# marcinp7/music-style-transfer

Hardware: AMD Instinct MI355X
Metric: style-transfer opt iters/sec (higher is better)
Workload: dtype f32; 1 GPU; one 30 s clip per GPU (BASELINE.json configs[1]): piano-roll C=4,R=16,T=4 (+percussion), full widths (980325 params), fwd+loss+bwd every step, Adam+StepLR every iter_size steps; clips_per_gpu=1, iter_size=2, hip_graph=True, graphs=one joint graph, accumulation=2 concurrent streams, launches_per_pass=71, parallelism=single GPU

## Files before the change

music-style-transfer_amd/csrc/loss_optim.hip:

```cpp
#include "mst_common.h"

#define LOSS_MAXBLK 256
#define NP_SUMS 7
#define N_TAPE_IN 16
#define SAVED_J 0
#define EPS_DIV 1e-7f

int64_t mst_loss_scratch_floats(void) { return 2 * LOSS_MAXBLK * 8 + 64; }

template <int NFEAT>
__device__ __forceinline__ void note_terms(const float* p, const float* t, float* acc) {
    const float pv = p[1], tv = t[1];
    const float m = tv > 0.f ? 1.f : 0.f;
    acc[0] += fminf(pv, tv);
    acc[1] += fmaxf(pv - tv, 0.f);
    acc[2] += fmaxf(tv - pv, 0.f);
    const float dv = tv - pv;
    acc[3] += dv * dv * m;
    const float dd = (p[0] - fminf(t[0], 6.f)) / 6.f;
    acc[4] += dd * dd * m;
    if (NFEAT == 5) {
        float bce = 0.f;
#pragma unroll
        for (int a = 2; a < 5; ++a) {
            const float lp = fmaxf(logf(p[a]), -100.f), lq = fmaxf(logf(1.f - p[a]), -100.f);
            bce -= t[a] * lp + (1.f - t[a]) * lq;
        }
        acc[5] += bce * m;
    }
    acc[6] += m;
}
// ... 92 lines not shown

__device__ __forceinline__ ChannelLeaves channel_tree(const Dual* in, bool pitched, bool normalize) {
    const Dual TP = in[0], FP = in[1], FN = in[2], SEV = in[3], SED = in[4];
    const Dual NM = pitched ? in[6] : in[5];
    ChannelLeaves o;
    const Dual prec = d_safe_div(TP, d_add(TP, FP));
    const Dual rec = d_safe_div(TP, d_add(TP, FN));
    const Dual f = d_cmul(d_safe_div(d_mul(prec, rec), d_add(prec, rec)), 2.f);
    o.notes = d_one_minus(f);
    o.vel = d_div(SEV, NM);
    o.dur = d_div(SED, NM);
    const Dual nv = d_safe_sqrt(d_add(d_mul(o.notes, d_sqr(o.notes)), d_mul(d_one_minus(o.notes), d_sqr(o.vel))));
    if (pitched) {
        o.acc = d_div(in[5], d_cmul(NM, 3.f));
        if (normalize) o.acc = d_tanh(o.acc);
        o.total = d_qmean3(o.dur, o.acc, nv);
    } else {
        o.acc = dl(0.f, 0.f);
        o.total = d_qmean2(o.dur, nv);
    }
    return o;
}

__global__ __launch_bounds__(64) void loss_tail_kernel(const float* scratch, int nblk_p, int nblk_u, int has_u,
                                                       const float* il, const float* it, int ni,
                                                       const float* mlg, const float* mt,
                                                       const float* bp, const float* bt, int normalize,
                                                       float* losses, float* saved, LossBatch lb,
                                                       float* gl_onehot, float* losses_out) {
    __shared__ float sums[N_TAPE_IN];
    const int tid = threadIdx.x;
    {
        const int64_t k = blockIdx.y;
        scratch += k * lb.tmp; il += k * lb.ws; it += k * lb.ws; mlg += k * lb.ws; mt += k * lb.ws; bp += k * lb.ws;
        bt += k * lb.ws; losses += k * lb.ws; saved += k * lb.ws;
        if (gl_onehot) gl_onehot += k * lb.ws;
        if (losses_out) losses_out += k * MST_N_LOSSES;
    }
    {
        float sp[8] = {0.f, 0.f, 0.f, 0.f, 0.f, 0.f, 0.f, 0.f}, su[8] = {0.f, 0.f, 0.f, 0.f, 0.f, 0.f, 0.f, 0.f};
        typedef float row4 __attribute__((ext_vector_type(4), aligned(4)));
        const row4* rp = reinterpret_cast<const row4*>(scratch);
        const row4* ru = reinterpret_cast<const row4*>(scratch + LOSS_MAXBLK * 8);
        const int nbu = has_u ? nblk_u : 0;
        for (int q = tid; q < nblk_p; q += 64) {
            const row4 x = rp[2 * q], y = rp[2 * q + 1];
            sp[0] += x.x; sp[1] += x.y; sp[2] += x.z; sp[3] += x.w; sp[4] += y.x; sp[5] += y.y; sp[6] += y.z;
        }
        for (int q = tid; q < nbu; q += 64) {
            const row4 x = ru[2 * q], y = ru[2 * q + 1];
            su[0] += x.x; su[1] += x.y; su[2] += x.z; su[3] += x.w; su[4] += y.x; su[5] += y.y; su[6] += y.z;
        }
#pragma unroll
        for (int k = 0; k < 7; ++k) { sp[k] = wave_sum(sp[k]); su[k] = wave_sum(su[k]); }
        if (tid == 0) {
#pragma unroll
            for (int k = 0; k < 7; ++k) sums[k] = sp[k];
#pragma unroll
            for (int k = 0; k < 5; ++k) sums[7 + k] = su[k];
            sums[12] = su[6];
        }
    }
    float v = 0.f;
    for (int j = tid; j < ni; j += 64) {
        const float x = il[j];
        v += fmaxf(x, 0.f) - x * it[j] + log1pf(expf(-fabsf(x)));
    }
    v = wave_sum(v);
    if (tid == 0) {
        sums[13] = v / (float)ni;
        const int tgt = mt[1] > mt[0] ? 1 : 0;
        const float mx = fmaxf(mlg[0], mlg[1]);
        const float lse = mx + logf(expf(mlg[0] - mx) + expf(mlg[1] - mx));
        sums[14] = lse - mlg[tgt];
        const float db = (bp[0] - bt[0]) / 150.f;
        sums[15] = db * db;
    }
    __syncthreads();
    if (tid >= N_TAPE_IN) return;
    Dual in[N_TAPE_IN];
#pragma unroll
    for (int j = 0; j < N_TAPE_IN; ++j) in[j] = dl(sums[j], j == tid ? 1.f : 0.f);
    Dual leaf[MST_N_LOSSES];
    bool present[MST_N_LOSSES];
#pragma unroll
    for (int k = 0; k < MST_N_LOSSES; ++k) { leaf[k] = dl(0.f, 0.f); present[k] = true; }
    const ChannelLeaves p = channel_tree(in, true, normalize != 0);
    leaf[MST_L_P_TOTAL] = p.total; leaf[MST_L_P_NOTES] = p.notes; leaf[MST_L_P_VELOCITY] = p.vel;
    leaf[MST_L_P_DURATION] = p.dur; leaf[MST_L_P_ACCIDENTALS] = p.acc;
    if (has_u) {
        const ChannelLeaves u = channel_tree(in + 7, false, normalize != 0);
        leaf[MST_L_U_TOTAL] = u.total; leaf[MST_L_U_NOTES] = u.notes; leaf[MST_L_U_VELOCITY] = u.vel;
        leaf[MST_L_U_DURATION] = u.dur;
        leaf[MST_L_CH_TOTAL] = d_qmean2(p.total, u.total);
    } else {
        present[MST_L_U_TOTAL] = present[MST_L_U_NOTES] = present[MST_L_U_VELOCITY] = present[MST_L_U_DURATION] = false;
        leaf[MST_L_CH_TOTAL] = p.total;
    }
    Dual li = in[13], lm = in[14];
    if (normalize) { li = d_tanh(li); lm = d_tanh(lm); }
    leaf[MST_L_SI_INSTRUMENTS] = li;
    leaf[MST_L_SI_MODE] = lm;
    leaf[MST_L_SI_BPM] = in[15];
    leaf[MST_L_SI_TOTAL] = d_qmean3(li, lm, in[15]);
    leaf[MST_L_TOTAL] = d_qmean2(leaf[MST_L_CH_TOTAL], leaf[MST_L_SI_TOTAL]);
#pragma unroll
    for (int k = 0; k < MST_N_LOSSES; ++k) {
        if (tid == 0) {
            const float v = present[k] ? leaf[k].v : __builtin_nanf("");
            losses[k] = v;
            if (losses_out) losses_out[k] = v;
            if (gl_onehot) gl_onehot[k] = k == MST_L_TOTAL ? 1.f : 0.f;
        }
        saved[SAVED_J + k * N_TAPE_IN + tid] = present[k] ? leaf[k].d : 0.f;
    }
}

__global__ __launch_bounds__(256) void loss_bwd_kernel(const float* pp, const float* pt, int64_t np, int nblk_p,
                                                       const float* up, const float* ut, int64_t nu, int nblk_u,
                                                       const float* il, const float* it, int ni,
                                                       const float* mlg, const float* mt, const float* bp, const float* bt,
                                                       const float* saved, const float* gl,
                                                       float* gp, float* gu, float* gi, float* gm, float* gb, LossBatch lb, float info_scale) {
    __shared__ float coef[N_TAPE_IN];
    __shared__ float tile_p[256 * 5], tile_t[256 * 5];
    {
        const int64_t k = blockIdx.y;
        pp += k * lb.ws; pt += k * lb.ext0; up += k * lb.ws; ut += k * lb.ext1;
        il += k * lb.ws; it += k * lb.ws; mlg += k * lb.ws; mt += k * lb.ws; bp += k * lb.ws; bt += k * lb.ws;
        saved += k * lb.ws; gl += k * lb.ws;
        gp += k * lb.grad; gu += k * lb.grad; gi += k * lb.grad; gm += k * lb.grad; gb += k * lb.grad;
    }
    if (threadIdx.x < N_TAPE_IN) {
        float gk[MST_N_LOSSES], sk[MST_N_LOSSES];
#pragma unroll
        for (int k = 0; k < MST_N_LOSSES; ++k) { gk[k] = gl[k]; sk[k] = saved[SAVED_J + k * N_TAPE_IN + threadIdx.x]; }
        float c = 0.f;
// ... 61 lines not shown
    } else {
        const float ci = coef[13] * info_scale, cm = coef[14] * info_scale, cb = coef[15] * info_scale;
        for (int j = threadIdx.x; j < ni; j += 256) gi[j] = ci * (1.f / (1.f + expf(-il[j])) - it[j]) / (float)ni;
        if (threadIdx.x == 0) {
            const int tgt = mt[1] > mt[0] ? 1 : 0;
            const float mx = fmaxf(mlg[0], mlg[1]);
            const float e0 = expf(mlg[0] - mx), e1 = expf(mlg[1] - mx);
            gm[0] = cm * (e0 / (e0 + e1) - (tgt == 0 ? 1.f : 0.f));
            gm[1] = cm * (e1 / (e0 + e1) - (tgt == 1 ? 1.f : 0.f));
            gb[0] = cb * 2.f * (bp[0] - bt[0]) / (150.f * 150.f);
        }
    }
}

static int blocks_for(int64_t n) {
    int64_t b = (n + 1023) / 1024;
    if (b < 1) b = 1;
    if (b > LOSS_MAXBLK) b = LOSS_MAXBLK;
    return (int)b;
}

int loss_fwd_batched(const float* pp, const float* pt, int64_t np, const float* up, const float* ut, int64_t nu, const float* il,
                     const float* it, int ni, const float* mlg, const float* mt, const float* bp, const float* bt, int normalize,
                     float* losses, float* saved, float* scratch, LossBatch lb, hipStream_t s, float* gl_onehot, float* losses_out) {
    if (!pp || !pt || !il || !it || !mlg || !mt || !bp || !bt || !losses || !saved || !scratch || np <= 0 || lb.clips < 1)
        return MST_ERR_ARG;
    const int has_u = (up && ut && nu > 0) ? 1 : 0;
    const int nbp = blocks_for(np), nbu = has_u ? blocks_for(nu) : 0;
    hipLaunchKernelGGL(loss_partials_kernel, dim3(nbp + nbu, lb.clips), dim3(256), 0, s, pp, pt, np, nbp, up, ut,
                       has_u ? nu : (int64_t)0, nbu, scratch, lb);
    hipLaunchKernelGGL(loss_tail_kernel, dim3(1, lb.clips), dim3(64), 0, s, (const float*)scratch, nbp, nbu, has_u, il, it,
                       ni, mlg, mt, bp, bt, normalize, losses, saved, lb, gl_onehot, losses_out);
    return hipGetLastError() == hipSuccess ? MST_OK : MST_ERR_LAUNCH;
}

int loss_bwd_batched(const float* pp, const float* pt, int64_t np, const float* up, const float* ut, int64_t nu, const float* il,
                     const float* it, int ni, const float* mlg, const float* mt, const float* bp, const float* bt,
                     const float* saved, const float* gl, float* gp, float* gu, float* gi, float* gm, float* gb, LossBatch lb,
                     hipStream_t s, float info_scale) {
    if (!pp || !pt || !saved || !gl || !gi || !gm || !gb || np <= 0 || lb.clips < 1) return MST_ERR_ARG;
    const int has_u = (up && ut && gu && nu > 0) ? 1 : 0;
    const int nbp = gp ? blocks_for(np) : 0, nbu = has_u ? blocks_for(nu) : 0;
    hipLaunchKernelGGL(loss_bwd_kernel, dim3(nbp + nbu + 1, lb.clips), dim3(256), 0, s, pp, pt, np, nbp, up, ut,
                       has_u ? nu : (int64_t)0, nbu, il, it, ni, mlg, mt, bp, bt, saved, gl, gp, gu, gi, gm, gb, lb, info_scale);
    return hipGetLastError() == hipSuccess ? MST_OK : MST_ERR_LAUNCH;
}

static const LossBatch ONE_CLIP = {1, 0, 0, 0, 0, 0};

int loss_blocks(int64_t n) { return blocks_for(n); }

int loss_fwd_partials(const float* pp, const float* pt, int64_t np, const float* up, const float* ut, int64_t nu, float* scratch,
                      hipStream_t s) {
    const int has_u = (up && ut && nu > 0) ? 1 : 0;
    const int nbp = blocks_for(np), nbu = has_u ? blocks_for(nu) : 0;
    hipLaunchKernelGGL(loss_partials_kernel, dim3(nbp + nbu, 1), dim3(256), 0, s, pp, pt, np, nbp, up, ut,
                       has_u ? nu : (int64_t)0, nbu, scratch, ONE_CLIP);
    return hipGetLastError() == hipSuccess ? MST_OK : MST_ERR_LAUNCH;
}

int loss_fwd_tail(int64_t np, int64_t nu, int has_u, const float* il, const float* it, int ni, const float* mlg, const float* mt,
                  const float* bp, const float* bt, int normalize, float* losses, float* saved, float* scratch, hipStream_t s,
                  float* gl_onehot, float* losses_out) {
    const int nbp = blocks_for(np), nbu = has_u ? blocks_for(nu) : 0;
    hipLaunchKernelGGL(loss_tail_kernel, dim3(1, 1), dim3(64), 0, s, (const float*)scratch, nbp, nbu, has_u, il, it,
                       ni, mlg, mt, bp, bt, normalize, losses, saved, ONE_CLIP, gl_onehot, losses_out);
    return hipGetLastError() == hipSuccess ? MST_OK : MST_ERR_LAUNCH;
}

extern "C" int32_t mst_total_loss_fwd(const float* pp, const float* pt, int64_t np, const float* up, const float* ut,
                                      int64_t nu, const float* il, const float* it, int32_t ni, const float* mlg,
                                      const float* mt, const float* bp, const float* bt, int32_t normalize,
                                      float* losses, float* saved, float* scratch, mst_stream stream) {
    return loss_fwd_batched(pp, pt, np, up, ut, nu, il, it, (int)ni, mlg, mt, bp, bt, (int)normalize, losses, saved, scratch,
                            ONE_CLIP, (hipStream_t)stream, nullptr, nullptr);
}

extern "C" int32_t mst_total_loss_bwd(const float* pp, const float* pt, int64_t np, const float* up, const float* ut,
                                      int64_t nu, const float* il, const float* it, int32_t ni, const float* mlg,
                                      const float* mt, const float* bp, const float* bt, const float* saved,
                                      const float* gl, float* gp, float* gu, float* gi, float* gm, float* gb,
                                      mst_stream stream) {
    return loss_bwd_batched(pp, pt, np, up, ut, nu, il, it, (int)ni, mlg, mt, bp, bt, saved, gl, gp, gu, gi, gm, gb, ONE_CLIP,
                            (hipStream_t)stream);
}

__device__ __forceinline__ void adam_advance(float* state, double lr0, double b1, double b2, int step_size, double gamma) {
    const int t = (int)state[0] + 1;
    const double lr = lr0 * pow(gamma, (double)((t - 1) / step_size));
// ... 1457 lines not shown
```

music-style-transfer_amd/csrc/mst_common.h:

```cpp
#pragma once
#include <hip/hip_runtime.h>
#include <stdint.h>

#include "../../include/mst_amd.h"

#ifndef MST_GLOBAL_AS
#define MST_GLOBAL_AS __attribute__((address_space(1)))
#endif
#ifndef MST_CONST_AS
#define MST_CONST_AS __attribute__((address_space(4)))
#endif
#ifndef MST_UNIFORM
#define MST_UNIFORM(x) __builtin_amdgcn_readfirstlane(x)
#endif
#ifndef MST_FAST_EXP
#define MST_FAST_EXP(x) __expf(x)
#define MST_FAST_RCP(x) __builtin_amdgcn_rcpf(x)
#define MST_PIN(x) asm volatile("" : "+v"(x))
#endif
#ifndef MST_PIN_SGPR
#if defined(__AMDGCN__)
#define MST_PIN_SGPR(p) asm volatile("" : "+s"(p))
#else
#define MST_PIN_SGPR(p) ((void)(p))
// ... 206 lines not shown
}


struct LinDesc {
    int32_t rows, K, N, act, xgrad, clips;
    int32_t x_space, x_ld; int64_t x_off, x_cs;
    int32_t y_ld; int64_t y_off, y_cs;
    int64_t gx_cs;
    int64_t w_off, b_off;
    int64_t slab_off, slab_stride, rows_per_split; int32_t splits;
    int32_t first[2];
};
int launch_lin_fwd(const LinDesc& d, Bases b, hipStream_t s);
int launch_lin_dx(const LinDesc& d, Bases b, int first, hipStream_t s);
int launch_lin_dw(const LinDesc& d, Bases b, hipStream_t s);
int lin_dw_tiles(const LinDesc& d);

struct RowLinDesc {
    int32_t rows, kin, nout, act, xgrad;
    int64_t x_off, y_off;
    int64_t w_off, b_off;
    int64_t slab_off; int32_t slab_stride, nblk;
    int32_t first;
};

struct CopyDesc { int64_t src_off, dst_off; int32_t na, nb, cols, src_sa, src_sb, dst_sa, dst_sb, first; };
struct FoldDesc { int32_t space, nrows, row_stride, ncols, col_stride, pad; int64_t part_off, sum_off ; };
int launch_copy_rows(const CopyDesc* dev, const CopyDesc& host, int backward, Bases b, hipStream_t s);
int launch_fold(const FoldDesc* dev, int spread, Bases b, hipStream_t s);
int launch_combine_phase(const CombineDesc* dev, int nblk, int which, Bases b, hipStream_t s, int count = 1, int mc4 = 0, int whole_small = 0);

struct SlabEntry { int64_t dst, src, stride; int32_t count, splits; int32_t reps; int64_t rep_stride; int32_t width, dst_ld; int32_t single;
                   int64_t base;  };
struct SlabBlock { int32_t entry, start; };

struct Sizes {
    int OC, PCE_IL, H, HB;
    int SE_L, SE_IL, SE_ML, SE_BL;
    int ME_BL, ME_BRL, ME_IL, ME_CW, MEL;
    int RH, PRE_BL, PRE_BRL, PRE_CL, PRE_IL, PRE_ML, PRE_BPL, URE_CL;
    int SIM_BL, NRF, SIM_SI, SIM_RI, SIM_SM, SIM_RM, SIM_SB, SIM_RB, NI;
    int PSA_SL, PSA_RL, PSA_IL, PSA_ML, USA_SL, USA_RL;
    int I, STYLE, BAR;
};
Sizes mst_sizes(const mst_dims& d);

// ... 2 lines not shown
int gemm_variant(const GemmDesc& g);
int launch_gemm(const GemmDesc* dev_descs, const int* dev_owner, int members, int blocks_per_clip, int clips, int mfma, Bases b, hipStream_t s,
                const GemmRiders* riders = nullptr);
int gemm_rider_blocks(const GemmRiders& r);
int gemm_tile_edge(int mfma);
int gemm_blocks(const GemmDesc& g, int mfma);
int launch_segred(const SegRedDesc* dev_descs, int members, int blocks_per_clip, int clips, int stage2_blocks, Bases b, hipStream_t s);
int launch_segred2(const SegRedDesc* dev_descs, int count, int stage2_blocks, Bases b, hipStream_t s);
int launch_lstm_transpose(const LstmDesc* dev_descs, int count, int maxH, int multi, Bases b, hipStream_t s);
int launch_lstm_fwd(const LstmDesc* dev_descs, int count, int maxB, int maxH, int multi, int small, Bases b, hipStream_t s);
int launch_lstm_bwd(const LstmDesc* dev_descs, int count, int maxB, int maxH, int multi, int small, Bases b, hipStream_t s);
bool lstm_small(int count, int maxB, int maxH);
int lstm_multi_blocks_per_cu();
int launch_combine_fwd(const CombineDesc* dev_descs, int count, int max_nblk, int all_small, int mc4, Bases b, hipStream_t s);
int launch_combine_bwd(const CombineDesc* dev_descs, int count, int max_nblk, int all_small, int mc4, Bases b, hipStream_t s);
int launch_me_sumsq(const NotesDesc* dev, const NotesDesc& host, int count, Bases b, hipStream_t s);
int launch_me_notes_fwd(const NotesDesc* dev, const NotesDesc& host, int count, Bases b, hipStream_t s);
int launch_me_bwd_reduce(const NotesDesc* dev, const NotesDesc& host, int count, Bases b, hipStream_t s);
int launch_me_notes_bwd(const NotesDesc* dev, const NotesDesc& host, int count, Bases b, hipStream_t s);
int launch_psa_notes_fwd(const NotesDesc* dev, const NotesDesc& host, int count, Bases b, hipStream_t s);
int launch_psa_notes_bwd(const NotesDesc* dev, const NotesDesc& host, int count, Bases b, hipStream_t s);
int psa_bwd_waves(int C);
struct LossBatch { int32_t clips; int64_t ws, grad, tmp, ext0, ext1; };
int loss_fwd_partials(const float* pp, const float* pt, int64_t np, const float* up, const float* ut, int64_t nu, float* scratch,
                      hipStream_t s);
int loss_fwd_tail(int64_t np, int64_t nu, int has_u, const float* il, const float* it, int ni, const float* mlg, const float* mt,
                  const float* bp, const float* bt, int normalize, float* losses, float* saved, float* scratch, hipStream_t s,
                  float* gl_onehot, float* losses_out);
int loss_blocks(int64_t n);
int loss_fwd_batched(const float* pp, const float* pt, int64_t np, const float* up, const float* ut, int64_t nu, const float* il,
                     const float* it, int ni, const float* mlg, const float* mt, const float* bp, const float* bt, int normalize,
                     float* losses, float* saved, float* scratch, LossBatch lb, hipStream_t s,
                     float* gl_onehot ,
                     float* losses_out );
int loss_bwd_batched(const float* pp, const float* pt, int64_t np, const float* up, const float* ut, int64_t nu, const float* il,
                     const float* it, int ni, const float* mlg, const float* mt, const float* bp, const float* bt,
                     const float* saved, const float* gl, float* gp, float* gu, float* gi, float* gm, float* gb, LossBatch lb,
                     hipStream_t s, float info_scale = 1.f );
int launch_roll_metrics(const float* pred, const float* target, int64_t n_groups, int64_t group_cells, int nfeat, int gpc,
                        int64_t pred_cs, int64_t tgt_cs, void* scratch, hipStream_t s);
struct EvalMetricsArgs {
    const void* part_p; int64_t slices_p, cells_p;
    const void* part_u; int64_t slices_u, cells_u;
    int32_t C, ni;
    const float *il, *it, *mlg, *mt, *bp, *bt;
    int64_t ws_stride;
    double* out;
};
int launch_eval_metrics_finish(const EvalMetricsArgs& a, int clips, hipStream_t s);
bool rowlin_supported(int kin, int nout);
int launch_rowlin_fwd(const RowLinDesc* dev, const RowLinDesc& host, int count, Bases b, hipStream_t s);
int launch_rowlin_bwd(const RowLinDesc* dev, const RowLinDesc& host, int count, Bases b, hipStream_t s);
int launch_slab_reduce(const SlabEntry* dev, const SlabBlock* blocks, int nblocks, Bases b, hipStream_t s);
struct ZeroChunk { int64_t off; int32_t len; int32_t pad; };
int launch_zero(const ZeroChunk* dev, int nchunks, int clips, float* grad_base, int64_t clip_stride, hipStream_t s);
bool notes_widths_supported(int W, int CW, int ML);

// ... 6 lines not shown
```

music-style-transfer_amd/csrc/notes.hip:

```cpp
#include "mst_common.h"

__device__ __forceinline__ float lrelu(float z) { return z > 0.f ? z : z * LEAKY; }
__device__ __forceinline__ float dlrelu(float y) { return y > 0.f ? 1.f : LEAKY; }

typedef float nt_f32x4 __attribute__((ext_vector_type(4)));
#define NT_ROW 66

__device__ __forceinline__ float wave_sum64(float v) {
#pragma unroll
    for (int o = 32; o > 0; o >>= 1) v += __shfl_xor(v, o);
    return v;
}

template <int N>
__device__ __forceinline__ void ld_vec(const float* p, float (&v)[N]) {
    static_assert(N % 4 == 0, "16-byte rows");
#pragma unroll
    for (int i = 0; i < N / 4; ++i) { const float4 t = reinterpret_cast<const float4*>(p)[i]; v[4 * i] = t.x; v[4 * i + 1] = t.y; v[4 * i + 2] = t.z; v[4 * i + 3] = t.w; }
}
template <int N>
__device__ __forceinline__ void st_vec(float* p, const float (&v)[N]) {
#pragma unroll
    for (int i = 0; i < N / 4; ++i) reinterpret_cast<float4*>(p)[i] = make_float4(v[4 * i], v[4 * i + 1], v[4 * i + 2], v[4 * i + 3]);
}
// ... 847 lines not shown
#pragma unroll
            for (int k = 0; k < KIN; ++k) z = fmaf(w_s[n * KIN + k], x[k], z);
            y[n] = rl_act(d.act, z, n);
        }
        rl_store<NOUT>(y0 + (int64_t)row * NOUT, y);
    }
}

template <int KIN, int NOUT>
__global__ __launch_bounds__(256) void rowlin_bwd_kernel(const RowLinDesc* __restrict__ dp, Bases b) {
    const RowLinDesc d = dp[blockIdx.y];
    constexpr int NACC = NOUT * KIN + NOUT;
    constexpr int RW = NOUT + KIN;
    constexpr int RP = 256 + 4;
    static_assert(NACC <= 256, "role count exceeds the workgroup");
    __shared__ float w_s[NOUT * KIN];
    __shared__ __attribute__((aligned(16))) float st[RW][RP];
    const int tid = threadIdx.x;
    for (int i = tid; i < NOUT * KIN; i += 256) w_s[i] = b.p[SP_PAR][d.w_off + i];
    const float* x0 = b.p[SP_WS] + d.x_off;
    const float* y0 = b.p[SP_WS] + d.y_off;
    const float* gy0 = b.p[SP_GRAD] + d.y_off;
    float* gx0 = b.p[SP_GRAD] + d.x_off;
    const int rn = tid < NOUT * KIN ? tid / KIN : tid - NOUT * KIN;
    const int rk = tid < NOUT * KIN ? NOUT + tid % KIN : -1;
    float wacc = 0.f;
    for (int base = blockIdx.x * 256; base < d.rows; base += gridDim.x * 256) {
        const int row = base + tid;
        __syncthreads();
        if (row < d.rows) {
            float x[KIN], y[NOUT], g[NOUT];
            rl_load<KIN>(x0 + (int64_t)row * KIN, x);
            rl_load<NOUT>(y0 + (int64_t)row * NOUT, y);
            rl_load<NOUT>(gy0 + (int64_t)row * NOUT, g);
#pragma unroll
            for (int n = 0; n < NOUT; ++n) { g[n] *= rl_dact(d.act, y[n], n); st[n][tid] = g[n]; }
#pragma unroll
            for (int k = 0; k < KIN; ++k) st[NOUT + k][tid] = x[k];
            if (d.xgrad) {
                float dx[KIN];
                if (d.first) {
#pragma unroll
                    for (int k = 0; k < KIN; ++k) dx[k] = 0.f;
                } else rl_load<KIN>(gx0 + (int64_t)row * KIN, dx);
#pragma unroll
                for (int k = 0; k < KIN; ++k) {
                    float a = 0.f;
#pragma unroll
                    for (int n = 0; n < NOUT; ++n) a = fmaf(g[n], w_s[n * KIN + k], a);
                    dx[k] += a;
                }
                rl_store<KIN>(gx0 + (int64_t)row * KIN, dx);
            }
        } else {
#pragma unroll
            for (int j = 0; j < NOUT + KIN; ++j) st[j][tid] = 0.f;
        }
// ... 40 lines not shown
```

music-style-transfer_amd/csrc/plan.hip:

```cpp
#include <algorithm>
#include <cmath>
#include <cstdio>
#include <cstdlib>
#include <cstring>
#include <map>
#include <string>
#include <array>
#include <vector>

#include "mst_common.h"

#define MST_ALIGN_UP(n) (((n) + 63) / 64 * 64)

static int mean_size(double a, double b, double factor = 1.0) { return (int)std::ceil(((a + b) / 2.0) * factor); }

Sizes mst_sizes(const mst_dims& d) {
    Sizes z{};
    z.I = d.instr; z.STYLE = d.style; z.BAR = d.bar; z.H = d.beat; z.HB = d.bar / 2; z.RH = d.rhythm;
    z.MEL = d.melody; z.NRF = d.nrf; z.NI = d.n_instruments;
    z.OC = mean_size(NF * NPF, d.beat);
    z.PCE_IL = mean_size(d.instr, d.beat);
    z.SE_L = mean_size(d.bar, d.style);
    z.SE_IL = mean_size(d.instr, d.style, .25);
    z.SE_ML = mean_size(2, d.style, .1);
// ... 203 lines not shown
struct Op { int stage; std::vector<Step> fwd, bwd; };

static int stage_idx(int stage) { return stage == MST_STAGE_EXTRACT ? 0 : stage == MST_STAGE_INFO ? 1 : 2; }

struct mst_plan {
    mst_dims d; Sizes z; ParamTable pt;
    DescTable<GemmDesc> gemms; DescTable<GatherDesc> gathers; DescTable<SegRedDesc> segreds; DescTable<LstmDesc> lstms;
    DescTable<CombineDesc> combines; DescTable<NotesDesc> notes; DescTable<RowLinDesc> rowlins;
    DescTable<ConvDesc> convs; DescTable<LinDesc> lins; DescTable<CopyDesc> copies; DescTable<FoldDesc> folds;
    std::vector<SlabEntry> slabs[3];
    std::vector<Op> ops;
    std::vector<Step> sched[2];
    std::vector<Step> sched_all[2];
    const std::vector<Step>& list(int mask, int backward) const { return mask == MST_STAGE_ALL ? sched_all[backward ? 1 : 0] : sched[backward ? 1 : 0]; }
    std::vector<int> s_gemm_owner; int* d_gemm_owner = nullptr;
    std::map<std::string, T> named;
    int64_t act_top = 0, tmp_top = 0;
    SlabEntry* d_slabs[3] = {nullptr, nullptr, nullptr};
    std::vector<SlabBlock> slab_blocks[3]; SlabBlock* d_slab_blocks[3] = {nullptr, nullptr, nullptr};
    std::vector<SlabEntry> slabs_all; SlabEntry* d_slabs_all = nullptr;
    std::vector<SlabBlock> slab_blocks_all; SlabBlock* d_slab_blocks_all = nullptr;
    bool slabs_all_ok = false;
    T t_losses, t_saved, t_gl; int64_t loss_scratch = 0;
    struct LossOps { int64_t pp, up, il, mlg, bp, it, mt, bt, losses, saved, gl, np, nu; } loss{};
    void resolve_loss() {
        auto at = [&](const char* n) { return named.at(n).off; };
        const bool U = d.has_unpitched != 0;
        loss = {at("pitched_pred"), U ? at("unpitched_pred") : 0, at("instruments_pred"), at("mode_pred"), at("bpm_pred"),
                at("used_instruments"), at("mode"), at("bpm_target"), t_losses.off, t_saved.off, t_gl.off,
                (int64_t)P() * NF * NPN, U ? (int64_t)Q() * NF * NUN : 0};
    }
    std::vector<ZeroChunk> zero_stage[3], zero_all;
    ZeroChunk* d_zero_stage[3] = {nullptr, nullptr, nullptr}; ZeroChunk* d_zero_all = nullptr;
    int err = 0;
    mst_plan_options opt{};
    int mfma = 0;
    int lstm_small_on = 1;

    bool tiled() const { return opt.tile_rows > 0; }
    bool mixes() const { return !mfma && !tiled() && opt.branches != 1 && !opt.no_merge; }
    int mc4() const { return d.C <= 4 ? 1 : 0; }
    int Rl() const { return tiled() ? opt.tile_rows : d.R; }
    int P() const { return d.C * Rl() * d.T; }
    int Q() const { return Rl() * d.T; }
    struct Xchg { int space; int64_t off; int32_t len; };
    std::vector<Xchg> xchgs;
// ... 67 lines not shown
    }
    GatherDesc reloc(GatherDesc g, int k) const {
        g.out_off += shift(SP_WS, k);
        for (int i = 0; i < g.nseg; ++i) g.seg[i].off += shift(g.seg[i].space, k);
        return g;
    }
    SegRedDesc reloc(SegRedDesc r, int k) const {
        r.src_off += shift(SP_GRAD, k); r.dst_off += shift(SP_GRAD, k); r.part_off += shift(SP_TMP, k); r.y_off += shift(SP_WS, k);
        return r;
    }
    LstmDesc reloc(LstmDesc l, int k) const {
        const int64_t a = shift(SP_WS, k), t = shift(SP_TMP, k);
        l.zx_off += a; l.out_off += a; l.gout_off += a; l.gzx_off += a;
        l.gates_off += t; l.c_off += t; l.hprev_off += t; l.tc_off += t; l.xch_off += t;
        return l;
    }
    CombineDesc reloc(CombineDesc c, int k) const {
        const int64_t a = shift(SP_WS, k), t = shift(SP_TMP, k);
        c.x_off += a; c.out_off += a; c.gx_off += a; c.gout_off += a; c.stats_off += t; c.part_off += t;
        return c;
    }
    RowLinDesc reloc(RowLinDesc r, int k) const {
        r.x_off += shift(SP_WS, k); r.y_off += shift(SP_WS, k); r.slab_off += shift(SP_TMP, k);
        return r;
    }
    NotesDesc reloc(NotesDesc n, int k) const {
        const int64_t a = shift(SP_WS, k), t = shift(SP_TMP, k);
        n.oct_off += a; n.deg_off += a; n.rt_oct_off += a; n.rt_deg_off += a; n.it_oct_off += a; n.it_deg_off += a; n.mel_off += a; n.g_mel_off += a; n.out_off += a; n.g_out_off += a; n.g_oct_off += a; n.g_deg_off += a;
        n.g_ml_off += a; n.x_off += shift(n.x_space, k); n.slab_off += t; n.part_off += t; n.stats_off += t;
        n.itp_oct_off += a; n.itp_deg_off += a; n.loss_saved_off += a; n.loss_gl_off += a;
        return n;
    }
    template <class F> void with_sched_table(int fam, F&& f) {
        switch (fam) {
        case F_GEMM: f(gemms); break;       case F_GATHER: f(gathers); break;     case F_SEGRED: f(segreds); break;
        case F_LSTM: f(lstms); break;       case F_COMB: f(combines); break;      case F_NOTES: f(notes); break;
        case F_ROWLIN: f(rowlins); break;   default: err = MST_ERR_UNSUPPORTED;
        }
    }

    static int64_t align(int64_t n) { return (n + 63) / 64 * 64; }
    T newT(int rows, int cols, const char* name = nullptr) {
        T t{act_top, rows, cols, cols};
        act_top += align((int64_t)rows * cols);
        if (name) named[name] = t;
        return t;
// ... 634 lines not shown
            n.bl_off != n.wl_off + (int64_t)NPF * (NPF * 6 + z.PSA_ML))
            err = MST_ERR_UNSUPPORTED;
        n.out_off = xp.off; n.g_out_off = xp.off;
        n.itp_oct_off = itp_x[0].off; n.itp_deg_off = itp_x[1].off;
        n.x_space = SP_EXT0; n.x_off = 0;
        n.loss_saved_off = t_saved.off; n.loss_gl_off = t_gl.off;
        const int nw = z.PSA_ML * z.MEL + z.PSA_ML + NPF * (NPF * 6 + z.PSA_ML) + NPF;
        n.nblk = psa_nblk; n.slab_stride = nw; n.slab_off = tmp((int64_t)nw * n.nblk);
        Op op; op.stage = AP;
        op.fwd.push_back(Step{K_PSA_F, (int)notes.host.size(), 1, 0, 0});
        op.bwd.push_back(Step{K_PSA_B, (int)notes.host.size(), 1, 0, 0});
        notes.host.push_back(n); ops.push_back(op);
        slabs[2].push_back(SlabEntry{n.wm_off, n.slab_off, nw, nw, n.nblk});
    }
    if (U) {
        m = "unpitched_style_applier";
        T usa_sl = linear(AP, style, true, m + ".style_linear", NF * z.USA_SL, ACT_LEAKY);
        T usa_rl = linear(AP, rhythm, true, m + ".rhythm_linear", z.USA_RL, ACT_LEAKY);
        T sl_view{usa_sl.off, NF, z.USA_SL, z.USA_SL};
        const int rsQ_F[4] = {Q_, NF, 1, 1};
        T ucat = gather(AP, rsQ_F, {seg(sl_view, 0, 1, 0, 0), seg(usa_rl, NF, 1, 0, 0)});
        T v = linear(AP, ucat, true, m + ".notes_linear", NUN * NUF * 4, ACT_LEAKY);
        T v_rows{v.off, Q_ * NF * NUN, NUF * 4, NUF * 4};
        rowlin(AP, v_rows, true, m + ".linear", NUF, ACT_SIGOUT, "unpitched_pred");
    }
    if (!widths_supported(z)) err = MST_ERR_UNSUPPORTED;
}

static void acc_add(std::vector<Acc>& v, int space, int64_t lo, int64_t len, bool w, bool accum = false, bool dense = true) {
    if (space != SP_WS && space != SP_GRAD && space != SP_TMP) return;
    if (len <= 0) return;
    Acc a{space, lo, lo + len, w}; a.accum = accum; a.dense = dense;
    v.push_back(a);
}

static void operand_acc(std::vector<Acc>& v, const Operand& o, int di, int dj, int ones) {
    switch (o.kind) {
    case OPK_DENSE: {
        const int64_t si = o.si < 0 ? -o.si : o.si, sj = o.sj < 0 ? -o.sj : o.sj;
        const int dj_eff = ones >= 0 ? dj - 1 : dj;
        acc_add(v, o.space, o.off, (int64_t)(di - 1) * si + (int64_t)(dj_eff > 0 ? dj_eff - 1 : 0) * sj + 1, false);
        break;
    }
    case OPK_ACTGRAD: {
        const int rows = o.transposed ? dj : di;
        acc_add(v, o.space, o.off, (int64_t)rows * o.ld, false);
        acc_add(v, o.space2, o.off2, (int64_t)rows * o.ld, false);
// ... 127 lines not shown
            if (s.kind == K_COPY_F) { acc_add(v, SP_WS, c.src_off, ss, false); acc_add(v, SP_WS, c.dst_off, ds, true); }
            else { acc_add(v, SP_GRAD, c.dst_off, ds, false); acc_add(v, SP_GRAD, c.src_off, ss, true, true, false); }
            break;
        }
        case K_FOLD: case K_SPREAD: {
            const FoldDesc& f = folds.host[s.first + i];
            const int64_t span = (int64_t)(f.nrows - 1) * f.row_stride + (int64_t)(f.ncols - 1) * f.col_stride + 1;
            acc_add(v, f.space, f.part_off, span, s.kind == K_SPREAD);
            acc_add(v, SP_TMP, f.sum_off, f.ncols, s.kind == K_FOLD);
            break;
        }
        case K_XCHG: {
            const Xchg& x = xchgs[s.first + i];
            acc_add(v, x.space, x.off, x.len, true);
            break;
        }
        case K_ROW_F: case K_ROW_B: {
            const RowLinDesc& r = tab(rowlins)[s.first + i];
            const int64_t nx = (int64_t)r.rows * r.kin, ny = (int64_t)r.rows * r.nout;
            acc_add(v, SP_WS, r.x_off, nx, false);
            acc_add(v, SP_WS, r.y_off, ny, s.kind == K_ROW_F);
            if (s.kind == K_ROW_B) {
                acc_add(v, SP_GRAD, r.y_off, ny, false);
                if (r.xgrad) acc_add(v, SP_GRAD, r.x_off, nx, true, true, true);
                acc_add(v, SP_TMP, r.slab_off, (int64_t)r.slab_stride * r.nblk, true);
            }
            break;
        }
        case K_ME_SQ: case K_ME_F: case K_ME_RED: case K_ME_B: {
            const NotesDesc& n = tab(notes)[s.first + i];
            const int64_t rows = (int64_t)n.C * n.Q, mel = (int64_t)n.Q * NF * NPN * n.W;
            const int64_t nparts = (int64_t)(n.C + 1) * n.nwc;
            acc_add(v, SP_WS, n.oct_off, rows * NOCT * n.W, false);
            acc_add(v, SP_WS, n.deg_off, rows * NDEG * n.W, false);
            if (s.kind == K_ME_SQ) acc_add(v, SP_TMP, n.part_off, nparts, true);
            else if (s.kind == K_ME_F) {
                acc_add(v, SP_TMP, n.part_off, nparts, false);
                acc_add(v, SP_TMP, n.stats_off, n.C + 1, true);
                acc_add(v, SP_WS, n.out_off, mel, true);
            } else if (s.kind == K_ME_RED) {
                acc_add(v, SP_WS, n.out_off, mel, false);
                acc_add(v, SP_GRAD, n.g_out_off, mel, false);
                acc_add(v, SP_TMP, n.part_off, nparts, true);
            } else {
                acc_add(v, SP_TMP, n.part_off, nparts, false);
                acc_add(v, SP_TMP, n.stats_off, n.C + 1, false);
// ... 646 lines not shown
    if ((mask & MST_STAGE_EXTRACT) && (!pitched || (p->d.has_unpitched && !unpitched))) return MST_ERR_ARG;
    Bases b = make_bases(p, params, gparams, ws, pitched, unpitched);
    b.flags = flags;
    {
        int e = run_pass(p, p->list(mask, 1), mask, b, (hipStream_t)stream);
        if (e) return e;
    }
    if ((mask & MST_STAGE_ALL) == MST_STAGE_ALL && p->slabs_all_ok)
        return launch_slab_reduce(p->d_slabs_all, p->d_slab_blocks_all, (int)p->slab_blocks_all.size(), b, (hipStream_t)stream) ? MST_ERR_LAUNCH : MST_OK;
    for (int s = 2; s >= 0; --s) {
        if (!((mask >> s) & 1)) continue;
        if (launch_slab_reduce(p->d_slabs[s], p->d_slab_blocks[s], (int)p->slab_blocks[s].size(), b, (hipStream_t)stream))
            return MST_ERR_LAUNCH;
    }
    return MST_OK;
}

extern "C" int32_t mst_backward(const mst_plan* p, int32_t mask, const float* params, float* gparams, float* ws,
                                const float* pitched, const float* unpitched, mst_stream stream) {
    return backward_impl(p, mask, params, gparams, ws, pitched, unpitched, stream, 0);
}

enum { LOSS_WHOLE, LOSS_PARTIALS, LOSS_TAIL };
static int loss_forward(const mst_plan* p, int what, float* ws, const float* pitched, const float* unpitched, float* losses, hipStream_t st) {
    const mst_plan::LossOps& o = p->loss;
    const bool U = p->d.has_unpitched != 0;
    const float *pp = ws + o.pp, *up = U ? ws + o.up : nullptr, *ut = U ? unpitched : nullptr;
    float* scratch = ws + p->arena(SP_TMP) + p->loss_scratch;
    if (what == LOSS_PARTIALS) return loss_fwd_partials(pp, pitched, o.np, up, ut, o.nu, scratch, st);
    if (what == LOSS_TAIL)
        return loss_fwd_tail(o.np, o.nu, U ? 1 : 0, ws + o.il, ws + o.it, p->z.NI, ws + o.mlg, ws + o.mt, ws + o.bp, ws + o.bt, 1,
                             ws + o.losses, ws + o.saved, scratch, st, ws + o.gl, losses);
    return loss_fwd_batched(pp, pitched, o.np, up, ut, o.nu, ws + o.il, ws + o.it, p->z.NI, ws + o.mlg, ws + o.mt, ws + o.bp, ws + o.bt, 1,
                            ws + o.losses, ws + o.saved, scratch, p->loss_batch(), st, ws + o.gl, losses);
}
static int loss_backward(const mst_plan* p, float* ws, const float* pitched, const float* unpitched, bool pitched_grad, const LossBatch& lb,
                         float info_scale, hipStream_t st) {
    const mst_plan::LossOps& o = p->loss;
    const bool U = p->d.has_unpitched != 0;
    float* g = ws + p->arena(SP_GRAD);
    return loss_bwd_batched(ws + o.pp, pitched, o.np, U ? ws + o.up : nullptr, U ? unpitched : nullptr, o.nu, ws + o.il, ws + o.it, p->z.NI,
                            ws + o.mlg, ws + o.mt, ws + o.bp, ws + o.bt, ws + o.saved, ws + o.gl, pitched_grad ? g + o.pp : nullptr,
                            U ? g + o.up : nullptr, g + o.il, g + o.mlg, g + o.bp, lb, st, info_scale);
}

extern "C" int32_t mst_train_iteration(const mst_plan* p, const float* params, float* gparams, float* ws,
                                       const float* pitched, const float* unpitched, float* losses, mst_stream stream) {
    if (!p || !params || !gparams || !ws || !pitched) return MST_ERR_ARG;
    hipStream_t st = (hipStream_t)stream;
    int e = p->zero_ride >= 0 ? 0 : mst_zero_grads(p, MST_STAGE_ALL, ws, stream);
    if (e) return e;
    if (p->d.has_unpitched && !unpitched) return MST_ERR_ARG;
    e = run_pass(p, p->list(MST_STAGE_ALL, 0), MST_STAGE_ALL, make_bases(p, params, nullptr, ws, pitched, unpitched), st, p->tags_in_zero, p->zero_ride);
    if (e) return e;
    e = loss_forward(p, LOSS_WHOLE, ws, pitched, unpitched, losses, st);
    if (e) return e;
    e = loss_backward(p, ws, pitched, unpitched, false , p->loss_batch(), 1.f, st);
    if (e) return e;
    e = backward_impl(p, MST_STAGE_ALL, params, gparams, ws, pitched, unpitched, stream, MST_BF_LOSS_FUSED);
    if (e) return e;
    return hipGetLastError() == hipSuccess ? MST_OK : MST_ERR_LAUNCH;
}

static int64_t eval_slices(const mst_plan* p, bool pitched) {
    return mst_roll_slices(pitched ? (int64_t)p->Q() * NF * NPN : (int64_t)p->Q() * NF * NUN);
}

extern "C" int64_t mst_eval_scratch_bytes(const mst_plan* p) {
    if (!p) return MST_ERR_ARG;
    if (p->tiled()) return MST_ERR_UNSUPPORTED;
    return 32 * (int64_t)p->K() * ((int64_t)p->d.C * eval_slices(p, true) + (p->d.has_unpitched ? eval_slices(p, false) : 0));
}

extern "C" int32_t mst_eval_iteration(const mst_plan* p, const float* params, float* ws, const float* pitched,
                                      const float* unpitched, float* losses, double* metrics, void* scratch, mst_stream stream) {
    if (!p || !params || !ws || !pitched || !metrics || !scratch || ((uintptr_t)metrics & 7) || ((uintptr_t)scratch & 7)) return MST_ERR_ARG;
    if (p->tiled()) return MST_ERR_UNSUPPORTED;
    if (p->d.has_unpitched && !unpitched) return MST_ERR_ARG;
    hipStream_t st = (hipStream_t)stream;
    int e = run_pass(p, p->list(MST_STAGE_ALL, 0), MST_STAGE_ALL, make_bases(p, params, nullptr, ws, pitched, unpitched), st);
    if (e) return e;
// ... 275 lines not shown
```

Measured before the change: 2917 iters/s.

## Fuse loss backward into loss tail and unpitched rowlin backward

The loss tail kernel now also writes the info, mode and BPM head gradients, using the saved tape derivatives. The unpitched rowlin backward kernel recomputes its output gradient from the saved loss coefficients and targets instead of loading a gradient written by a separate loss backward kernel. Together these drop the separate loss_bwd launch from the training iteration when unpitched fusion applies. The cost is extra per-row arithmetic in the rowlin backward, a more complex dependency setup, and reliance on the plan marking the fused rowlin correctly.

```diff
diff --git a/music-style-transfer_amd/csrc/loss_optim.hip b/music-style-transfer_amd/csrc/loss_optim.hip
--- a/music-style-transfer_amd/csrc/loss_optim.hip
+++ b/music-style-transfer_amd/csrc/loss_optim.hip
@@ -7,6 +7,19 @@
 #define EPS_DIV 1e-7f
 
 int64_t mst_loss_scratch_floats(void) { return 2 * LOSS_MAXBLK * 8 + 64; }
+
+struct LossTail {
+    const float *il, *it; int ni;
+    const float *mlg, *mt, *bp, *bt; int normalize;
+    float *losses, *saved, *gl_onehot, *losses_out, *gi, *gm, *gb;
+    __device__ __forceinline__ void shift(int64_t k, const LossBatch& lb) {
+        il += k * lb.ws; it += k * lb.ws; mlg += k * lb.ws; mt += k * lb.ws; bp += k * lb.ws; bt += k * lb.ws;
+        losses += k * lb.ws; saved += k * lb.ws;
+        if (gl_onehot) gl_onehot += k * lb.ws;
+        if (losses_out) losses_out += k * MST_N_LOSSES;
+        if (gi) { gi += k * lb.grad; gm += k * lb.grad; gb += k * lb.grad; }
+    }
+};
 
 template <int NFEAT>
 __device__ __forceinline__ void note_terms(const float* p, const float* t, float* acc) {
@@ -145,62 +158,9 @@
     return o;
 }
 
-__global__ __launch_bounds__(64) void loss_tail_kernel(const float* scratch, int nblk_p, int nblk_u, int has_u,
-                                                       const float* il, const float* it, int ni,
-                                                       const float* mlg, const float* mt,
-                                                       const float* bp, const float* bt, int normalize,
-                                                       float* losses, float* saved, LossBatch lb,
-                                                       float* gl_onehot, float* losses_out) {
-    __shared__ float sums[N_TAPE_IN];
-    const int tid = threadIdx.x;
-    {
-        const int64_t k = blockIdx.y;
-        scratch += k * lb.tmp; il += k * lb.ws; it += k * lb.ws; mlg += k * lb.ws; mt += k * lb.ws; bp += k * lb.ws;
-        bt += k * lb.ws; losses += k * lb.ws; saved += k * lb.ws;
-        if (gl_onehot) gl_onehot += k * lb.ws;
-        if (losses_out) losses_out += k * MST_N_LOSSES;
-    }
-    {
-        float sp[8] = {0.f, 0.f, 0.f, 0.f, 0.f, 0.f, 0.f, 0.f}, su[8] = {0.f, 0.f, 0.f, 0.f, 0.f, 0.f, 0.f, 0.f};
-        typedef float row4 __attribute__((ext_vector_type(4), aligned(4)));
-        const row4* rp = reinterpret_cast<const row4*>(scratch);
-        const row4* ru = reinterpret_cast<const row4*>(scratch + LOSS_MAXBLK * 8);
-        const int nbu = has_u ? nblk_u : 0;
-        for (int q = tid; q < nblk_p; q += 64) {
-            const row4 x = rp[2 * q], y = rp[2 * q + 1];
-            sp[0] += x.x; sp[1] += x.y; sp[2] += x.z; sp[3] += x.w; sp[4] += y.x; sp[5] += y.y; sp[6] += y.z;
-        }
-        for (int q = tid; q < nbu; q += 64) {
-            const row4 x = ru[2 * q], y = ru[2 * q + 1];
-            su[0] += x.x; su[1] += x.y; su[2] += x.z; su[3] += x.w; su[4] += y.x; su[5] += y.y; su[6] += y.z;
-        }
-#pragma unroll
-        for (int k = 0; k < 7; ++k) { sp[k] = wave_sum(sp[k]); su[k] = wave_sum(su[k]); }
-        if (tid == 0) {
-#pragma unroll
-            for (int k = 0; k < 7; ++k) sums[k] = sp[k];
-#pragma unroll
-            for (int k = 0; k < 5; ++k) sums[7 + k] = su[k];
-            sums[12] = su[6];
-        }
-    }
-    float v = 0.f;
-    for (int j = tid; j < ni; j += 64) {
-        const float x = il[j];
-        v += fmaxf(x, 0.f) - x * it[j] + log1pf(expf(-fabsf(x)));
-    }
-    v = wave_sum(v);
-    if (tid == 0) {
-        sums[13] = v / (float)ni;
-        const int tgt = mt[1] > mt[0] ? 1 : 0;
-        const float mx = fmaxf(mlg[0], mlg[1]);
-        const float lse = mx + logf(expf(mlg[0] - mx) + expf(mlg[1] - mx));
-        sums[14] = lse - mlg[tgt];
-        const float db = (bp[0] - bt[0]) / 150.f;
-        sums[15] = db * db;
-    }
-    __syncthreads();
-    if (tid >= N_TAPE_IN) return;
+__device__ __forceinline__ float loss_tail_leaves(const float* sums, int tid, int has_u, const LossTail& a) {
+    const int normalize = a.normalize;
+    float *losses = a.losses, *saved = a.saved, *gl_onehot = a.gl_onehot, *losses_out = a.losses_out;
     Dual in[N_TAPE_IN];
 #pragma unroll
     for (int j = 0; j < N_TAPE_IN; ++j) in[j] = dl(sums[j], j == tid ? 1.f : 0.f);
@@ -236,6 +196,72 @@
             if (gl_onehot) gl_onehot[k] = k == MST_L_TOTAL ? 1.f : 0.f;
         }
         saved[SAVED_J + k * N_TAPE_IN + tid] = present[k] ? leaf[k].d : 0.f;
+    }
+    return leaf[MST_L_TOTAL].d;
+}
+
+__global__ __launch_bounds__(64) void loss_tail_kernel(const float* scratch, int nblk_p, int nblk_u, int has_u, LossBatch lb, LossTail a) {
+    __shared__ float sums[N_TAPE_IN];
+    const int tid = threadIdx.x;
+    scratch += (int64_t)blockIdx.y * lb.tmp;
+    a.shift(blockIdx.y, lb);
+    const float *il = a.il, *it = a.it, *mlg = a.mlg, *mt = a.mt, *bp = a.bp, *bt = a.bt;
+    const int ni = a.ni;
+    {
+        float sp[8] = {0.f, 0.f, 0.f, 0.f, 0.f, 0.f, 0.f, 0.f}, su[8] = {0.f, 0.f, 0.f, 0.f, 0.f, 0.f, 0.f, 0.f};
+        typedef float row4 __attribute__((ext_vector_type(4), aligned(4)));
+        const row4* rp = reinterpret_cast<const row4*>(scratch);
+        const row4* ru = reinterpret_cast<const row4*>(scratch + LOSS_MAXBLK * 8);
+        const int nbu = has_u ? nblk_u : 0;
+        for (int q = tid; q < nblk_p; q += 64) {
+            const row4 x = rp[2 * q], y = rp[2 * q + 1];
+            sp[0] += x.x; sp[1] += x.y; sp[2] += x.z; sp[3] += x.w; sp[4] += y.x; sp[5] += y.y; sp[6] += y.z;
+        }
+        for (int q = tid; q < nbu; q += 64) {
+            const row4 x = ru[2 * q], y = ru[2 * q + 1];
+            su[0] += x.x; su[1] += x.y; su[2] += x.z; su[3] += x.w; su[4] += y.x; su[5] += y.y; su[6] += y.z;
+        }
+#pragma unroll
+        for (int k = 0; k < 7; ++k) { sp[k] = wave_sum(sp[k]); su[k] = wave_sum(su[k]); }
+        if (tid == 0) {
+#pragma unroll
+            for (int k = 0; k < 7; ++k) sums[k] = sp[k];
+#pragma unroll
+            for (int k = 0; k < 5; ++k) sums[7 + k] = su[k];
+            sums[12] = su[6];
+        }
+    }
+    float v = 0.f;
+    for (int j = tid; j < ni; j += 64) {
+        const float x = il[j];
+        v += fmaxf(x, 0.f) - x * it[j] + log1pf(expf(-fabsf(x)));
+    }
+    v = wave_sum(v);
+    if (tid == 0) {
+        sums[13] = v / (float)ni;
+        const int tgt = mt[1] > mt[0] ? 1 : 0;
+        const float mx = fmaxf(mlg[0], mlg[1]);
+        const float lse = mx + logf(expf(mlg[0] - mx) + expf(mlg[1] - mx));
+        sums[14] = lse - mlg[tgt];
+        const float db = (bp[0] - bt[0]) / 150.f;
+        sums[15] = db * db;
+    }
+    __syncthreads();
+    float c_info = 0.f;
+    if (tid < N_TAPE_IN) c_info += 1.f * loss_tail_leaves(sums, tid, has_u, a);
+    if (!a.gi) return;
+    __syncthreads();
+    if (tid >= 13 && tid < N_TAPE_IN) sums[tid] = c_info;
+    __syncthreads();
+    const float ci = sums[13] * 1.f, cm = sums[14] * 1.f, cb = sums[15] * 1.f;
+    for (int j = tid; j < ni; j += 64) a.gi[j] = ci * (1.f / (1.f + expf(-il[j])) - it[j]) / (float)ni;
+    if (tid == 0) {
+        const int tgt = mt[1] > mt[0] ? 1 : 0;
+        const float mx = fmaxf(mlg[0], mlg[1]);
+        const float e0 = expf(mlg[0] - mx), e1 = expf(mlg[1] - mx);
+        a.gm[0] = cm * (e0 / (e0 + e1) - (tgt == 0 ? 1.f : 0.f));
+        a.gm[1] = cm * (e1 / (e0 + e1) - (tgt == 1 ? 1.f : 0.f));
+        a.gb[0] = cb * 2.f * (bp[0] - bt[0]) / (150.f * 150.f);
     }
 }
 
@@ -343,15 +369,18 @@
 
 int loss_fwd_batched(const float* pp, const float* pt, int64_t np, const float* up, const float* ut, int64_t nu, const float* il,
                      const float* it, int ni, const float* mlg, const float* mt, const float* bp, const float* bt, int normalize,
-                     float* losses, float* saved, float* scratch, LossBatch lb, hipStream_t s, float* gl_onehot, float* losses_out) {
+                     float* losses, float* saved, float* scratch, LossBatch lb, hipStream_t s, float* gl_onehot, float* losses_out,
+                     const LossHeadGrads* heads) {
     if (!pp || !pt || !il || !it || !mlg || !mt || !bp || !bt || !losses || !saved || !scratch || np <= 0 || lb.clips < 1)
         return MST_ERR_ARG;
+    if (heads && (!heads->gi || !heads->gm || !heads->gb)) return MST_ERR_ARG;
     const int has_u = (up && ut && nu > 0) ? 1 : 0;
     const int nbp = blocks_for(np), nbu = has_u ? blocks_for(nu) : 0;
+    const LossTail t{il, it, ni, mlg, mt, bp, bt, normalize, losses, saved, gl_onehot, losses_out,
+                     heads ? heads->gi : nullptr, heads ? heads->gm : nullptr, heads ? heads->gb : nullptr};
     hipLaunchKernelGGL(loss_partials_kernel, dim3(nbp + nbu, lb.clips), dim3(256), 0, s, pp, pt, np, nbp, up, ut,
                        has_u ? nu : (int64_t)0, nbu, scratch, lb);
-    hipLaunchKernelGGL(loss_tail_kernel, dim3(1, lb.clips), dim3(64), 0, s, (const float*)scratch, nbp, nbu, has_u, il, it,
-                       ni, mlg, mt, bp, bt, normalize, losses, saved, lb, gl_onehot, losses_out);
+    hipLaunchKernelGGL(loss_tail_kernel, dim3(1, lb.clips), dim3(64), 0, s, (const float*)scratch, nbp, nbu, has_u, lb, t);
     return hipGetLastError() == hipSuccess ? MST_OK : MST_ERR_LAUNCH;
 }
 
@@ -384,8 +413,8 @@
                   const float* bp, const float* bt, int normalize, float* losses, float* saved, float* scratch, hipStream_t s,
                   float* gl_onehot, float* losses_out) {
     const int nbp = blocks_for(np), nbu = has_u ? blocks_for(nu) : 0;
-    hipLaunchKernelGGL(loss_tail_kernel, dim3(1, 1), dim3(64), 0, s, (const float*)scratch, nbp, nbu, has_u, il, it,
-                       ni, mlg, mt, bp, bt, normalize, losses, saved, ONE_CLIP, gl_onehot, losses_out);
+    const LossTail t{il, it, ni, mlg, mt, bp, bt, normalize, losses, saved, gl_onehot, losses_out, nullptr, nullptr, nullptr};
+    hipLaunchKernelGGL(loss_tail_kernel, dim3(1, 1), dim3(64), 0, s, (const float*)scratch, nbp, nbu, has_u, ONE_CLIP, t);
     return hipGetLastError() == hipSuccess ? MST_OK : MST_ERR_LAUNCH;
 }
 
diff --git a/music-style-transfer_amd/csrc/mst_common.h b/music-style-transfer_amd/csrc/mst_common.h
--- a/music-style-transfer_amd/csrc/mst_common.h
+++ b/music-style-transfer_amd/csrc/mst_common.h
@@ -252,6 +252,9 @@
     int64_t w_off, b_off;
     int64_t slab_off; int32_t slab_stride, nblk;
     int32_t first;
+    int32_t loss;
+    int32_t tgt_space; int64_t tgt_off;
+    int64_t loss_saved_off, loss_gl_off;
 };
 
 struct CopyDesc { int64_t src_off, dst_off; int32_t na, nb, cols, src_sa, src_sb, dst_sa, dst_sb, first; };
@@ -300,6 +303,7 @@
 int launch_psa_notes_bwd(const NotesDesc* dev, const NotesDesc& host, int count, Bases b, hipStream_t s);
 int psa_bwd_waves(int C);
 struct LossBatch { int32_t clips; int64_t ws, grad, tmp, ext0, ext1; };
+struct LossHeadGrads { float *gi, *gm, *gb; };
 int loss_fwd_partials(const float* pp, const float* pt, int64_t np, const float* up, const float* ut, int64_t nu, float* scratch,
                       hipStream_t s);
 int loss_fwd_tail(int64_t np, int64_t nu, int has_u, const float* il, const float* it, int ni, const float* mlg, const float* mt,
@@ -310,7 +314,8 @@
                      const float* it, int ni, const float* mlg, const float* mt, const float* bp, const float* bt, int normalize,
                      float* losses, float* saved, float* scratch, LossBatch lb, hipStream_t s,
                      float* gl_onehot ,
-                     float* losses_out );
+                     float* losses_out ,
+                     const struct LossHeadGrads* heads = nullptr);
 int loss_bwd_batched(const float* pp, const float* pt, int64_t np, const float* up, const float* ut, int64_t nu, const float* il,
                      const float* it, int ni, const float* mlg, const float* mt, const float* bp, const float* bt,
                      const float* saved, const float* gl, float* gp, float* gu, float* gi, float* gm, float* gb, LossBatch lb,
diff --git a/music-style-transfer_amd/csrc/notes.hip b/music-style-transfer_amd/csrc/notes.hip
--- a/music-style-transfer_amd/csrc/notes.hip
+++ b/music-style-transfer_amd/csrc/notes.hip
@@ -893,6 +893,21 @@
     const float* y0 = b.p[SP_WS] + d.y_off;
     const float* gy0 = b.p[SP_GRAD] + d.y_off;
     float* gx0 = b.p[SP_GRAD] + d.x_off;
+    constexpr bool CAN_LOSS = KIN == 8 && NOUT == 2;
+    __shared__ float coef_s[CAN_LOSS ? 8 : 1];
+    const bool loss = CAN_LOSS && (b.flags & MST_BF_LOSS_FUSED) != 0 && d.loss != 0;
+    if constexpr (CAN_LOSS) if (loss && tid < 6) {
+        const float* saved = b.p[SP_WS] + d.loss_saved_off;
+        const float* gl = b.p[SP_WS] + d.loss_gl_off;
+        float gk[MST_N_LOSSES], sk[MST_N_LOSSES];
+#pragma unroll
+        for (int q = 0; q < MST_N_LOSSES; ++q) { gk[q] = gl[q]; sk[q] = saved[q * 16 + 7 + tid]; }
+        float a = 0.f;
+#pragma unroll
+        for (int q = 0; q < MST_N_LOSSES; ++q) a += gk[q] != 0.f ? gk[q] * sk[q] : 0.f;
+        coef_s[tid] = a;
+    }
+    const float* t0 = loss ? b.p[d.tgt_space] + d.tgt_off : nullptr;
     const int rn = tid < NOUT * KIN ? tid / KIN : tid - NOUT * KIN;
     const int rk = tid < NOUT * KIN ? NOUT + tid % KIN : -1;
     float wacc = 0.f;
@@ -903,7 +918,22 @@
             float x[KIN], y[NOUT], g[NOUT];
             rl_load<KIN>(x0 + (int64_t)row * KIN, x);
             rl_load<NOUT>(y0 + (int64_t)row * NOUT, y);
-            rl_load<NOUT>(gy0 + (int64_t)row * NOUT, g);
+            bool have_g = false;
+            if constexpr (CAN_LOSS) {
+                if (loss) {
+                    const float cTP = coef_s[0], cFP = coef_s[1], cFN = coef_s[2], cSEV = coef_s[3], cSED = coef_s[4];
+                    const float t_0 = t0[(int64_t)row * 2], tv = t0[(int64_t)row * 2 + 1];
+                    const float pv = y[1], p0 = y[0];
+                    const float m = tv > 0.f ? 1.f : 0.f;
+                    float gv = cTP * (pv < tv ? 1.f : (pv == tv ? 0.5f : 0.f));
+                    gv += cFP * (pv - tv > 0.f ? 1.f : 0.f) - cFN * (tv - pv > 0.f ? 1.f : 0.f);
+                    gv -= cSEV * 2.f * (tv - pv) * m;
+                    g[1] = gv;
+                    g[0] = cSED * 2.f * (p0 - fminf(t_0, 6.f)) * (1.f / 36.f) * m;
+                    have_g = true;
+                }
+            }
+            if (!have_g) rl_load<NOUT>(gy0 + (int64_t)row * NOUT, g);
 #pragma unroll
             for (int n = 0; n < NOUT; ++n) { g[n] *= rl_dact(d.act, y[n], n); st[n][tid] = g[n]; }
 #pragma unroll
diff --git a/music-style-transfer_amd/csrc/plan.hip b/music-style-transfer_amd/csrc/plan.hip
--- a/music-style-transfer_amd/csrc/plan.hip
+++ b/music-style-transfer_amd/csrc/plan.hip
@@ -249,6 +249,7 @@
     std::vector<SlabBlock> slab_blocks_all; SlabBlock* d_slab_blocks_all = nullptr;
     bool slabs_all_ok = false;
     T t_losses, t_saved, t_gl; int64_t loss_scratch = 0;
+    bool unpitched_loss_fused = false;
     struct LossOps { int64_t pp, up, il, mlg, bp, it, mt, bt, losses, saved, gl, np, nu; } loss{};
     void resolve_loss() {
         auto at = [&](const char* n) { return named.at(n).off; };
@@ -362,6 +363,7 @@
     }
     RowLinDesc reloc(RowLinDesc r, int k) const {
         r.x_off += shift(SP_WS, k); r.y_off += shift(SP_WS, k); r.slab_off += shift(SP_TMP, k);
+        if (r.loss) { r.tgt_off += shift(r.tgt_space, k); r.loss_saved_off += shift(SP_WS, k); r.loss_gl_off += shift(SP_WS, k); }
         return r;
     }
     NotesDesc reloc(NotesDesc n, int k) const {
@@ -1042,7 +1044,14 @@
         T ucat = gather(AP, rsQ_F, {seg(sl_view, 0, 1, 0, 0), seg(usa_rl, NF, 1, 0, 0)});
         T v = linear(AP, ucat, true, m + ".notes_linear", NUN * NUF * 4, ACT_LEAKY);
         T v_rows{v.off, Q_ * NF * NUN, NUF * 4, NUF * 4};
+        const size_t before = rowlins.host.size();
         rowlin(AP, v_rows, true, m + ".linear", NUF, ACT_SIGOUT, "unpitched_pred");
+        if (rowlins.host.size() > before) {
+            RowLinDesc& r = rowlins.host.back();
+            r.loss = 1; r.tgt_space = SP_EXT1; r.tgt_off = 0;
+            r.loss_saved_off = t_saved.off; r.loss_gl_off = t_gl.off;
+            unpitched_loss_fused = true;
+        }
     }
     if (!widths_supported(z)) err = MST_ERR_UNSUPPORTED;
 }
@@ -1216,6 +1225,7 @@
             acc_add(v, SP_WS, r.y_off, ny, s.kind == K_ROW_F);
             if (s.kind == K_ROW_B) {
                 acc_add(v, SP_GRAD, r.y_off, ny, false);
+                if (r.loss) { acc_add(v, SP_WS, r.loss_saved_off, MST_LOSS_SAVED, false); acc_add(v, SP_WS, r.loss_gl_off, 64, false); }
                 if (r.xgrad) acc_add(v, SP_GRAD, r.x_off, nx, true, true, true);
                 acc_add(v, SP_TMP, r.slab_off, (int64_t)r.slab_stride * r.nblk, true);
             }
@@ -1908,7 +1918,8 @@
 }
 
 enum { LOSS_WHOLE, LOSS_PARTIALS, LOSS_TAIL };
-static int loss_forward(const mst_plan* p, int what, float* ws, const float* pitched, const float* unpitched, float* losses, hipStream_t st) {
+static int loss_forward(const mst_plan* p, int what, float* ws, const float* pitched, const float* unpitched, float* losses, hipStream_t st,
+                        bool head_grads = false) {
     const mst_plan::LossOps& o = p->loss;
     const bool U = p->d.has_unpitched != 0;
     const float *pp = ws + o.pp, *up = U ? ws + o.up : nullptr, *ut = U ? unpitched : nullptr;
@@ -1917,8 +1928,10 @@
     if (what == LOSS_TAIL)
         return loss_fwd_tail(o.np, o.nu, U ? 1 : 0, ws + o.il, ws + o.it, p->z.NI, ws + o.mlg, ws + o.mt, ws + o.bp, ws + o.bt, 1,
                              ws + o.losses, ws + o.saved, scratch, st, ws + o.gl, losses);
+    float* g = ws + p->arena(SP_GRAD);
+    const LossHeadGrads heads{g + o.il, g + o.mlg, g + o.bp};
     return loss_fwd_batched(pp, pitched, o.np, up, ut, o.nu, ws + o.il, ws + o.it, p->z.NI, ws + o.mlg, ws + o.mt, ws + o.bp, ws + o.bt, 1,
-                            ws + o.losses, ws + o.saved, scratch, p->loss_batch(), st, ws + o.gl, losses);
+                            ws + o.losses, ws + o.saved, scratch, p->loss_batch(), st, ws + o.gl, losses, head_grads ? &heads : nullptr);
 }
 static int loss_backward(const mst_plan* p, float* ws, const float* pitched, const float* unpitched, bool pitched_grad, const LossBatch& lb,
                          float info_scale, hipStream_t st) {
@@ -1939,10 +1952,12 @@
     if (p->d.has_unpitched && !unpitched) return MST_ERR_ARG;
     e = run_pass(p, p->list(MST_STAGE_ALL, 0), MST_STAGE_ALL, make_bases(p, params, nullptr, ws, pitched, unpitched), st, p->tags_in_zero, p->zero_ride);
     if (e) return e;
-    e = loss_forward(p, LOSS_WHOLE, ws, pitched, unpitched, losses, st);
+    e = loss_forward(p, LOSS_WHOLE, ws, pitched, unpitched, losses, st, true);
     if (e) return e;
-    e = loss_backward(p, ws, pitched, unpitched, false , p->loss_batch(), 1.f, st);
-    if (e) return e;
+    if (p->d.has_unpitched && !p->unpitched_loss_fused) {
+        e = loss_backward(p, ws, pitched, unpitched, false, p->loss_batch(), 1.f, st);
+        if (e) return e;
+    }
     e = backward_impl(p, MST_STAGE_ALL, params, gparams, ws, pitched, unpitched, stream, MST_BF_LOSS_FUSED);
     if (e) return e;
     return hipGetLastError() == hipSuccess ? MST_OK : MST_ERR_LAUNCH;
```

New measurement: 2942 iters/s (median of 6 runs). No clear change (+0.8%).
